# francescobrigante/Audio-Style-Transfer

Measured on AMD Instinct MI355X. Metric: audio-seconds/sec/node (train step, 4s@22.05kHz pairs), higher is better.
Workload: dtype bf16; 1 GPU; configs[1]: batch=8 4 s clips per GPU (S=2, x=(B,S,2,287,597)), full train2 step: STFT + CQT front-end from resident waveforms, encoders+decoder+discriminator, all losses, D and G phases, grad clip, Adam; global_batch=8, parallelism=dp1, hip_graph=True, dp_semantics=per-rank BN and batch-coupled losses

## Files before the change

### audio-style-transfer_amd/ast_amd/_lib.py

```python
from __future__ import annotations

import ctypes as C
import os

import torch

_HERE = os.path.dirname(os.path.abspath(__file__))
LIB_PATH = os.environ.get("AST_HIP_LIB") or os.path.join(_HERE, "libast_hip.so")

F32, BF16 = 0, 1
MAX_TAPS = 9
IGEMM_ACCUMULATE, IGEMM_RELU, IGEMM_WS_ZEROED, IGEMM_STATS, IGEMM_BN_SUMS, IGEMM_BN_NO_RELU, IGEMM_PER_IMAGE = (1 << b for b in range(7))
IGEMM_SLOTS_SHIFT, IGEMM_DET = 8, 4096

vp, i32, i64, f32 = C.c_void_p, C.c_int32, C.c_int64, C.c_float


class Gather(C.Structure):
    _fields_ = [(n, i32) for n in ("N", "Hs", "Ws", "Cs", "Hm", "Wm", "sh", "sw", "oh", "ow", "Hd", "Wd", "Cd",
                                   "dsh", "dsw", "doh", "dow", "ntaps", "wtaps")] + [("tap", i32 * MAX_TAPS)]


class WeightDesc(C.Structure):
    _fields_ = [("w", vp), ("u", vp), ("v", vp), ("sigma", vp), ("scratch", vp), ("wf", vp), ("wb", vp)] + \
# ... 10 lines not shown
    "ast_igemm": ([vp, vp, vp, vp, C.POINTER(Gather), i32, i32, vp, C.c_long, vp], i32),
    "ast_igemm_plan": ([C.POINTER(Gather), i32, C.POINTER(i32 * 5)], i32),
    "ast_pconv_variant": ([C.POINTER(Gather), i32, C.POINTER(i32 * 4)], i32),
    "ast_igemm_ws_floats": ([C.POINTER(Gather), i32], C.c_long),
    "ast_wgrad": ([vp, vp, vp, C.POINTER(Gather), i32, vp], i32),
    "ast_skinny_gemm": ([vp, vp, vp, vp, i32, i32, i32, i32, i32, i32, vp], i32),
    "ast_skinny_gemm_ex": ([vp, vp, vp, vp, i32, i32, i32, i32, i32, i32, vp, vp, f32, C.c_uint64, vp, vp], i32),
    "ast_bigk_gemm": ([vp, vp, vp, vp, i32, i32, i32, i32, vp], i32),
    "ast_bign_dgrad": ([vp, vp, vp, i32, i32, i32, i32, vp], i32),
    "ast_linear_wgrad": ([vp, vp, vp, vp, i32, i32, i32, i32, i32, vp], i32),
    "ast_linear_wgrad_batched": ([vp, i32, i32, vp], i32),
    "ast_linear_wgrad_batched_host": ([vp, i32, i32, vp], i32),
    "ast_nchw_to_nhwc": ([vp, vp, i32, i32, i32, i32, i64, i64, i64, i32, i32, vp], i32),
    "ast_nhwc_to_nchw": ([vp, vp, i32, i32, i32, i32, i32, i32, vp], i32),
    "ast_cast": ([vp, i32, vp, i32, i64, vp], i32),
    "ast_weights_prepare_t": ([vp, vp, i32, i32, i32, vp, i32, vp], i32),
    "ast_sn_scratch_floats": ([i32, i32], C.c_long),
    "ast_weight_grads_flush_t": ([vp, vp, i32, vp], i32),
    "ast_dropout_fwd": ([vp, vp, vp, i64, f32, C.c_uint64, vp, vp], i32),
    "ast_weight_grad_unpack": ([vp, i32, vp, vp, vp, vp, vp, i32, i32, i32, i32, i32, i32, i32, vp, vp], i32),
    "ast_chan_stats": ([vp, vp, i32, i32, i32, i32, i32, vp], i32),
    "ast_norm_finalize": ([vp, i32, vp, i32, i32, i32, i32, i32, vp, vp, vp, vp, i32, f32, vp, vp, vp, vp, C.c_long, vp], i32),
    "ast_affine_act": ([vp, vp, vp, vp, vp, vp, vp, i32, i32, i32, i32, i32, vp], i32),
    "ast_bn_apply_fwd": ([vp, vp, vp, vp, i32, C.c_long, vp, vp, vp, vp, vp, vp, f32, vp, vp, f32, vp, vp, i32, i32, i32, i32, i32, i32, vp], i32),
    "ast_bn_apply_bwd": ([vp, vp, vp, vp, vp, vp, i32, C.c_long, vp, vp, vp, vp, vp, vp, vp, vp, vp, vp, vp, vp, vp, vp, i32, i32, i32, i32, i32, i32, vp], i32),
    "ast_norm_bwd_sums": ([vp, vp, vp, vp, vp, i32, i32, i32, i32, i32, i32, vp], i32),
    "ast_norm_bwd_sums_pre": ([vp, vp, vp, vp, vp, i32, i32, i32, i32, i32, i32, vp, vp, vp, vp, vp], i32),
    "ast_norm_bwd_apply_pre": ([vp, vp, vp, vp, vp, vp, vp, vp, i32, i32, i32, i32, i32, vp, vp, vp, vp, vp], i32),
    "ast_norm_bwd_finalize": ([vp, i32, i32, i32, i32, i32, vp, vp, vp, vp, vp, vp, vp, vp, vp, vp, vp, vp, vp], i32),
    "ast_norm_bwd_finalize_n": ([vp, i32, i32, i32, i32, i32, vp, vp, vp, vp, vp, vp, vp, vp, vp, vp, vp, vp, C.c_long, vp], i32),
    "ast_igemm_bn": ([vp, vp, vp, vp, C.POINTER(Gather), i32, i32, vp, C.c_long, vp, vp, vp, vp], i32),
# ... 238 lines not shown
```

### audio-style-transfer_amd/ast_amd/layers.py

```python
from __future__ import annotations

import contextlib
import ctypes as C
import os

import torch
import torch.nn as nn

from . import config, ops, streams
from ._lib import LinWg, WeightDesc, check, dcode, lib, ptr, stream
from .ops import PackedWeight, pad8


class WeightBank:

    def __init__(self):
        self.specs = []
        self.entries: list[PackedWeight] = []
        self._key = None
        self._keys = {}
        self._flush_pending = False
        self._flush_stream = None
        self._lin_deferred = []
        self._pinned = []
        self._pin_pool = None
        self._pin_used = 0
        self._conv_dirty = False
        self._slab_recs = []
        self._conv_deferred = []
        self._defer_streams = []
        self._pool_flushed = False
        self._wait_lane = None
        self.d_train = self.d_eval = None
        self._dev_consts = {}
        self._packed = {}
        self.hold = False

    def add(self, weight, kind, dtype_fn, u=None, v=None, bias=None, rows=None):
        self.specs.append((weight, kind, dtype_fn, u, v, bias, rows))
        self.entries.append(PackedWeight())
        return self.entries[-1]

    def _const_dev(self, payload: bytes, dtype, dev):
        key = (payload, dtype, str(dev))
        t = self._dev_consts.get(key)
        if t is None:
            t = self._dev_consts[key] = torch.frombuffer(bytearray(payload), dtype=dtype).to(dev)
        return t
# ... 58 lines not shown
            grad_ptr = None
            if training:
                e.dwp, e.replicas, e.slab = None, rep, slab
                if sz:
                    e.dwp = self.dw_arena[off:off + sz]
                    off += sz
                    grad_ptr = ops.acc_grad(w).data_ptr() + 4 * w_off
            descs.append(WeightDesc(w=w.data_ptr() + 4 * w_off, u=ptr(u), v=ptr(v), sigma=ptr(e.sigma), scratch=ptr(e.scratch),
                                    wf=ptr(e.wf), wb=ptr(e.wb), Co=Co, Ci=Ci, KK=KK, s_co=s_co, s_ci=s_ci, Cop=e.Cop, Cip=e.Cip,
                                    power_iter=1 if training else 0, dwp=ptr(e.dwp), grad=grad_ptr, inner=ptr(e.gtmp),
                                    dwp_from_wb=1 if kind == "convT" else 0, dwp_replicas=(1 if slab else rep) if training else 1))
            dts.append(dcode(dt))
            self.max_co = max(self.max_co, Co)
            self.max_cols = max(self.max_cols, Ci * KK)
            self.max_packed = max(self.max_packed, n)
        tl = []
        for wi, e in enumerate(self.entries):
            for co0 in range(0, e.Cop, 32):
                for ci0 in range(0, e.Cip, 32):
                    tl += [wi, co0, ci0, 0]
        if self._pin_pool is None:
            self._pin_pool = torch.empty(256 * 1024, dtype=torch.uint8, pin_memory=True)
        import array
        self.ntiles = len(tl) // 4
        self.d_tiles = self._const_dev(array.array("i", tl).tobytes(), torch.int32, dev)
        arr = (WeightDesc * len(descs))(*descs)
        dev_descs = self._const_dev(bytes(arr), torch.uint8, dev)
        if training:
            self.d_train = dev_descs
        else:
            self.d_eval = dev_descs
        self.d_dtypes = self._const_dev(array.array("i", dts).tobytes(), torch.int32, dev)
        self._keys[training] = self._signature(training)

    def prepare(self, training: bool):
        if self.hold:
            return
        training = bool(training) and torch.is_grad_enabled()
        if self._keys.get(training) != self._signature(training):
            self._build(training)
        d = self.d_train if training else self.d_eval
        from . import _lib as _L
        if _L.PROFILE_CALLS is not None:
            _L.NEXT_BYTES = sum(e.Co * e.Ci * e.KK * 4 + 2 * e.wf.numel() * e.wf.element_size() for e in self.entries)
        check(lib().ast_weights_prepare_t(ptr(d), ptr(self.d_dtypes), len(self.entries), self.max_co, self.max_cols,
                                          ptr(self.d_tiles), self.ntiles, stream()), "ast_weights_prepare_t")

    def defer_linear_wgrad(self, pw, dy, x):
        self._lin_deferred.append((pw, dy, x))
        self.request_flush(conv=False)

    def defer_conv_wgrad(self, dy, src, dwp, g, replicas, pw):
        self._conv_deferred.append((dy, src, dwp, g, replicas, pw))
        if not any(b is self for b in _DeferPool.banks):
            _DeferPool.banks.append(self)

    def slab_used(self, pw):
        return next((n for p, n in self._slab_recs if p is pw), 0)

    def note_slab(self, pw, slices):
        for i, (p, n) in enumerate(self._slab_recs):
# ... 4 lines not shown

    def _sum_slabs(self):
        recs, self._slab_recs = self._slab_recs, []
        for i in range(0, len(recs), 48):
            part = recs[i:i + 48]
            n = len(part)
            bases = (C.c_void_p * n)(*[pw.dwp.data_ptr() for pw, _ in part])
            sizes = (C.c_int64 * n)(*[pw.dwp.numel() // pw.replicas for pw, _ in part])
            slabs = (C.c_int32 * n)(*[sl for _, sl in part])
            check(lib().ast_slab_sum(bases, sizes, slabs, n, stream()), "ast_slab_sum")

    def _flush_conv_kernels(self, side):
        with (torch.cuda.stream(side) if side is not None else contextlib.nullcontext()):
            if self._slab_recs:
                self._sum_slabs()
            if config.deterministic:
                ws = ops.det_ws(self.ntiles, self.d_tiles.device)
                check(lib().ast_weight_grads_flush_det(ptr(self.d_train), ptr(self.d_tiles), self.ntiles, ptr(ws), ws.numel(), stream()),
                      "ast_weight_grads_flush_det")
                return
            check(lib().ast_weight_grads_flush_t(ptr(self.d_train), ptr(self.d_tiles), self.ntiles, stream()),
                  "ast_weight_grads_flush_t")

    def _side_stream(self, origin):
        if self._flush_stream is None:
            self._flush_stream = torch.cuda.Stream(device=self.d_tiles.device)
        if not any(s is self._flush_stream for s in _ParallelFlush.pending):
            streams.fork(self._flush_stream, origin)
            _ParallelFlush.pending.append(self._flush_stream)
        return self._flush_stream

    def _launch_deferred(self, origin):
        items, self._conv_deferred = self._conv_deferred, []
        cur = torch.cuda.current_stream()
        k = max(1, min(config.wgrad_defer_streams, len(items)))
        if k > 1 and cur != origin:
# ... 20 lines not shown
    def request_flush(self, conv=True):
        self._conv_dirty = self._conv_dirty or conv
        if not self._flush_pending:
            self._flush_pending = True
            torch.autograd.Variable._execution_engine.queue_callback(self._flush)

    def _flush(self):
        self._flush_pending = False
        if ops._WgradStream.stream is not None and ops._WgradStream.dirty:
            ops._WgradStream.dirty = False
            streams.join(torch.cuda.current_stream(), ops._WgradStream.stream)
        if self._conv_dirty:
            self._conv_dirty = False
            from . import _lib as _L
            if _L.PROFILE_CALLS is not None:
                _L.NEXT_BYTES = sum((e.dwp.numel() * 4 if e.dwp is not None else 0) + 3 * e.Co * e.Ci * e.KK * 4 for e in self.entries if e.dwp is not None)
            side, origin = None, torch.cuda.current_stream()
            if _ParallelFlush.active:
                if config.wgrad_defer_pool and self._conv_deferred and len(_DeferPool.banks) > 1:
                    _DeferPool.launch_all(origin)
                side = self._side_stream(origin)
            if self._pool_flushed:
                self._pool_flushed = False
            else:
                with (torch.cuda.stream(side) if side is not None else contextlib.nullcontext()):
                    if self._conv_deferred:
                        self._launch_deferred(origin)
                    if self._wait_lane is not None:
                        torch.cuda.current_stream().wait_stream(self._wait_lane)
                        self._wait_lane = None
                self._flush_conv_kernels(side)
# ... 282 lines not shown
```

### audio-style-transfer_amd/csrc/weights.hip

```cpp
#include <type_traits>
#include "ast_common.h"
#include "../../include/ast_hip.h"

namespace {

__device__ __forceinline__ size_t woff(const ast_weight_desc_t& d, int co, int ci, int tap) {
  return (size_t)co * d.s_co + (size_t)ci * d.s_ci + tap;
}

constexpr int RZ = 32;
__global__ __launch_bounds__(256) void sn_wt_u_kernel(const ast_weight_desc_t* __restrict__ descs) {
  const ast_weight_desc_t d = descs[blockIdx.y];
  if (!d.u || !d.power_iter) return;
  const int ncols = d.Ci * d.KK;
  const int rows_per = (d.Co + RZ - 1) / RZ;
  const int c0 = blockIdx.z * rows_per, c1 = min(d.Co, c0 + rows_per);
  if (c0 >= c1) return;
  float* part = d.scratch + d.Co + (size_t)ncols * (1 + blockIdx.z);
  if (d.s_ci == d.KK && (ncols & 3) == 0 && (d.s_co & 3) == 0 && (((uintptr_t)d.w) & 15) == 0) {
    const int j4 = blockIdx.x * 256 + threadIdx.x;
    if (j4 >= (ncols >> 2)) return;
    f32x4 acc4 = {0.f, 0.f, 0.f, 0.f};
    for (int co = c0; co < c1; ++co) {
      const f32x4 w4 = *reinterpret_cast<const f32x4*>(d.w + (size_t)co * d.s_co + j4 * 4);
// ... 107 lines not shown
__device__ __forceinline__ bool tile_is_full(const ast_weight_desc_t& d, int co0, int ci0) {
  return co0 + TL <= d.Co && ci0 + TL <= d.Ci;
}
__device__ __forceinline__ bool master_vec_ok(const ast_weight_desc_t& d, const float* base) {
  const int inner = d.s_co >= d.s_ci ? d.s_ci : d.s_co, outer = d.s_co >= d.s_ci ? d.s_co : d.s_ci;
  return inner == d.KK && (outer & 3) == 0 && (((uintptr_t)base) & 15) == 0;
}

template <int KKC>
__device__ __forceinline__ void tile_load_master(const ast_weight_desc_t& d, const float* __restrict__ base, int co0, int ci0,
                                                 float* __restrict__ L, float scale) {
  const int KK = KKC > 0 ? KKC : d.KK;
  const bool co_outer = d.s_co >= d.s_ci;
  const int run = TL * KK;
  if (KKC > 0 && tile_is_full(d, co0, ci0) && master_vec_ok(d, base)) {
    const int run4 = run >> 2;
    for (int idx = threadIdx.x; idx < TL * run4; idx += 256) {
      const int o = idx / run4, r4 = idx - o * run4;
      const size_t off = co_outer ? (size_t)(co0 + o) * d.s_co + (size_t)ci0 * d.s_ci : (size_t)(ci0 + o) * d.s_ci + (size_t)co0 * d.s_co;
      const f32x4 v4 = *reinterpret_cast<const f32x4*>(base + off + r4 * 4);
#pragma unroll
      for (int e = 0; e < 4; ++e) {
        const int r = r4 * 4 + e;
        const int in = r / KK, tap = r - in * KK;
        const int co_l = co_outer ? o : in, ci_l = co_outer ? in : o;
        L[(tap * TL + co_l) * LP + ci_l] = v4[e] * scale;
      }
    }
    return;
  }
  for (int idx = threadIdx.x; idx < TL * run; idx += 256) {
    const int o = idx / run, r = idx - o * run;
    const int in = r / KK, tap = r - in * KK;
    const int co = co_outer ? co0 + o : co0 + in, ci = co_outer ? ci0 + in : ci0 + o;
    const float v = (co < d.Co && ci < d.Ci) ? base[(size_t)co * d.s_co + (size_t)ci * d.s_ci + tap] * scale : 0.f;
    L[(tap * TL + (co - co0)) * LP + (ci - ci0)] = v;
  }
}

template <typename T, int KKC>
__device__ __forceinline__ void tile_store_packed(const ast_weight_desc_t& d, int co0, int ci0, const float* __restrict__ L) {
// ... 50 lines not shown
    const float inv = 1.f / fmaxf(nrm, 1e-12f);
    sigma = nrm * nrm * inv;
    for (int i = threadIdx.x; i < d.Co; i += 256) d.u[i] = d.scratch[i] * inv;
  } else {
    float q = 0.f;
    for (int i = threadIdx.x; i < d.Co; i += 256) q += d.scratch[i] * d.u[i];
    sigma = block_sum(q, red);
  }
  if (threadIdx.x == 0) d.sigma[0] = sigma;
  __syncthreads();
}

template <int KKC>
__device__ __forceinline__ void pack_tile_body(const ast_weight_desc_t& d, const WTile& tl, int dtype, float* __restrict__ L) {
  const int KK = KKC > 0 ? KKC : d.KK;
  tile_load_master<KKC>(d, d.w, tl.co0, tl.ci0, L, 1.f / d.sigma[0]);
  __syncthreads();
  if (dtype == AST_BF16) tile_store_packed<bf16_t, KKC>(d, tl.co0, tl.ci0, L); else tile_store_packed<float, KKC>(d, tl.co0, tl.ci0, L);
  const int nrep = d.dwp_replicas > 1 ? d.dwp_replicas : 1;
  const size_t rstride = (size_t)d.Cop * KK * d.Cip;
  if (d.dwp && d.power_iter && KKC > 0 && tile_is_full(d, tl.co0, tl.ci0) && (d.Cip & 3) == 0 && (d.Cop & 3) == 0) {
    const f32x4 z = {0.f, 0.f, 0.f, 0.f};
    for (int idx = threadIdx.x; idx < TL * KK * 8; idx += 256) {
      const int q = idx & 7, row = idx >> 3;
      const int out_l = row / KK, tap = row - out_l * KK;
      float* p = d.dwp_from_wb ? d.dwp + ((size_t)(tl.ci0 + out_l) * KK + tap) * d.Cop + tl.co0 : d.dwp + ((size_t)(tl.co0 + out_l) * KK + tap) * d.Cip + tl.ci0;
      for (int r = 0; r < nrep; ++r) *reinterpret_cast<f32x4*>(p + r * rstride + q * 4) = z;
    }
  } else if (d.dwp && d.power_iter) {
    for (int idx = threadIdx.x; idx < TL * KK * TL; idx += 256) {
      const int in_l = idx & (TL - 1), row = idx >> 5;
      const int out_l = row / KK, tap = row - out_l * KK;
      for (int r = 0; r < nrep; ++r) {
        float* base = d.dwp + r * rstride;
        if (d.dwp_from_wb) { const int ci = tl.ci0 + out_l, co = tl.co0 + in_l; if (ci < d.Cip && co < d.Cop) base[((size_t)ci * KK + tap) * d.Cop + co] = 0.f; }
        else { const int co = tl.co0 + out_l, ci = tl.ci0 + in_l; if (co < d.Cop && ci < d.Cip) base[((size_t)co * KK + tap) * d.Cip + ci] = 0.f; }
      }
    }
  }
}

__global__ __launch_bounds__(256) void pack_tiles_kernel(const ast_weight_desc_t* __restrict__ descs, const int* __restrict__ dtypes,
                                                          const WTile* __restrict__ tiles) {
  __shared__ float L[9 * TL * LP];
  const WTile tl = tiles[blockIdx.x];
  const ast_weight_desc_t d = descs[tl.w];
  const int dt = dtypes[tl.w];
  if (d.KK == 9) pack_tile_body<9>(d, tl, dt, L);
  else if (d.KK == 1) pack_tile_body<1>(d, tl, dt, L);
  else pack_tile_body<0>(d, tl, dt, L);
}

template <int KKC>
__device__ __forceinline__ void tile_load_dwp(const ast_weight_desc_t& d, int co0, int ci0, float* __restrict__ G) {
  const int KK = KKC > 0 ? KKC : d.KK;
  const int nrep = d.dwp_replicas > 1 ? d.dwp_replicas : 1;
  const size_t rstride = (size_t)d.Cop * KK * d.Cip;
  if (KKC > 0 && tile_is_full(d, co0, ci0) && (d.Cip & 3) == 0 && (d.Cop & 3) == 0) {
    for (int idx = threadIdx.x; idx < TL * KK * 8; idx += 256) {
      const int q = idx & 7, row = idx >> 3;
      const int out_l = row / KK, tap = row - out_l * KK;
      const float* p = d.dwp_from_wb ? d.dwp + ((size_t)(ci0 + out_l) * KK + tap) * d.Cop + co0 : d.dwp + ((size_t)(co0 + out_l) * KK + tap) * d.Cip + ci0;
      f32x4 v4 = *reinterpret_cast<const f32x4*>(p + q * 4);
      if (nrep == 8) {
        f32x4 t[7];
#pragma unroll
        for (int r = 0; r < 7; ++r) t[r] = *reinterpret_cast<const f32x4*>(p + (r + 1) * rstride + q * 4);
        v4 = ((v4 + t[0]) + (t[1] + t[2])) + ((t[3] + t[4]) + (t[5] + t[6]));
      } else {
        for (int r = 1; r < nrep; ++r) v4 += *reinterpret_cast<const f32x4*>(p + r * rstride + q * 4);
      }
#pragma unroll
      for (int e = 0; e < 4; ++e) {
        const int in_l = q * 4 + e;
        const int co_l = d.dwp_from_wb ? in_l : out_l, ci_l = d.dwp_from_wb ? out_l : in_l;
        G[(tap * TL + co_l) * LP + ci_l] = v4[e];
      }
    }
    return;
  }
  for (int idx = threadIdx.x; idx < TL * KK * TL; idx += 256) {
    const int in_l = idx & (TL - 1), row = idx >> 5;
    const int out_l = row / KK, tap = row - out_l * KK;
    float v = 0.f;
    int co_l, ci_l;
    bool ok;
    size_t off;
    if (d.dwp_from_wb) { ci_l = out_l; co_l = in_l; const int ci = ci0 + ci_l, co = co0 + co_l; ok = ci < d.Ci && co < d.Co; off = ((size_t)ci * KK + tap) * d.Cop + co; }
    else { co_l = out_l; ci_l = in_l; const int co = co0 + co_l, ci = ci0 + ci_l; ok = co < d.Co && ci < d.Ci; off = ((size_t)co * KK + tap) * d.Cip + ci; }
    if (ok) {
      if (nrep == 8) {
        float t[8];
#pragma unroll
        for (int r = 0; r < 8; ++r) t[r] = d.dwp[r * rstride + off];
        v = ((t[0] + t[1]) + (t[2] + t[3])) + ((t[4] + t[5]) + (t[6] + t[7]));
      } else {
        for (int r = 0; r < nrep; ++r) v += d.dwp[r * rstride + off];
      }
    }
    G[(tap * TL + co_l) * LP + ci_l] = v;
  }
}

template <bool DET = false>
__global__ __launch_bounds__(256) void flush_inner_tiles_kernel(const ast_weight_desc_t* __restrict__ descs, const WTile* __restrict__ tiles,
                                                                float* __restrict__ part) {
  __shared__ float G[9 * TL * LP];
  __shared__ float red[17];
  const WTile tl = tiles[blockIdx.x];
  const ast_weight_desc_t d = descs[tl.w];
  if (!d.dwp || !d.u) {
    if constexpr (DET) { if (threadIdx.x == 0) part[blockIdx.x] = 0.f; }
    return;
  }
  float q = 0.f;
  auto body = [&](auto kkc) __attribute__((always_inline)) {
    constexpr int KKC = decltype(kkc)::value;
    const int KK = KKC > 0 ? KKC : d.KK;
    tile_load_dwp<KKC>(d, tl.co0, tl.ci0, G);
    __syncthreads();
    const bool co_outer = d.s_co >= d.s_ci;
    const int run = TL * KK;
    if (KKC > 0 && tile_is_full(d, tl.co0, tl.ci0) && master_vec_ok(d, d.w)) {
      const int run4 = run >> 2;
      for (int idx = threadIdx.x; idx < TL * run4; idx += 256) {
        const int o = idx / run4, r4 = idx - o * run4;
        const size_t off = co_outer ? (size_t)(tl.co0 + o) * d.s_co + (size_t)tl.ci0 * d.s_ci : (size_t)(tl.ci0 + o) * d.s_ci + (size_t)tl.co0 * d.s_co;
        const f32x4 w4 = *reinterpret_cast<const f32x4*>(d.w + off + r4 * 4);
#pragma unroll
        for (int e = 0; e < 4; ++e) {
          const int r = r4 * 4 + e;
          const int in = r / KK, tap = r - in * KK;
          const int co_l = co_outer ? o : in, ci_l = co_outer ? in : o;
          q += G[(tap * TL + co_l) * LP + ci_l] * w4[e];
        }
      }
      return;
    }
    for (int idx = threadIdx.x; idx < TL * run; idx += 256) {
      const int o = idx / run, r = idx - o * run;
      const int in = r / KK, tap = r - in * KK;
      const int co_l = co_outer ? o : in, ci_l = co_outer ? in : o;
      const int co = tl.co0 + co_l, ci = tl.ci0 + ci_l;
      if (co < d.Co && ci < d.Ci) q += G[(tap * TL + co_l) * LP + ci_l] * d.w[(size_t)co * d.s_co + (size_t)ci * d.s_ci + tap];
    }
  };
  if (d.KK == 9) body(std::integral_constant<int, 9>{});
  else if (d.KK == 1) body(std::integral_constant<int, 1>{});
  else body(std::integral_constant<int, 0>{});
  q = block_sum(q, red);
  if constexpr (DET) {
    if (threadIdx.x == 0) part[blockIdx.x] = q / d.sigma[0];
  } else {
    if (threadIdx.x == 0 && q != 0.f) unsafeAtomicAdd(d.inner, q / d.sigma[0]);
  }
}

__global__ __launch_bounds__(256) void inner_sum_det_kernel(const ast_weight_desc_t* __restrict__ descs, const WTile* __restrict__ tiles,
                                                            const float* __restrict__ part, int ntiles) {
  const int t = blockIdx.x * 256 + threadIdx.x;
  if (t >= ntiles) return;
  const int w = tiles[t].w;
  if (t > 0 && tiles[t - 1].w == w) return;
  const ast_weight_desc_t d = descs[w];
  if (!d.dwp || !d.u) return;
  float v = 0.f;
  for (int i = t; i < ntiles && tiles[i].w == w; ++i) v += part[i];
  d.inner[0] = v;
}

__global__ __launch_bounds__(256) void flush_unpack_tiles_kernel(const ast_weight_desc_t* __restrict__ descs, const WTile* __restrict__ tiles) {
  __shared__ float G[9 * TL * LP];
  const WTile tl = tiles[blockIdx.x];
  const ast_weight_desc_t d = descs[tl.w];
  if (!d.dwp || !d.grad) return;
  const float inner = d.u ? d.inner[0] : 0.f;
  const float inv_sigma = d.u ? 1.f / d.sigma[0] : 1.f;
  auto body = [&](auto kkc) __attribute__((always_inline)) {
    constexpr int KKC = decltype(kkc)::value;
    const int KK = KKC > 0 ? KKC : d.KK;
    tile_load_dwp<KKC>(d, tl.co0, tl.ci0, G);
    __syncthreads();
    const bool co_outer = d.s_co >= d.s_ci;
    const int run = TL * KK;
    if (KKC > 0 && tile_is_full(d, tl.co0, tl.ci0) && master_vec_ok(d, d.grad)) {
      const int run4 = run >> 2;
      for (int idx = threadIdx.x; idx < TL * run4; idx += 256) {
        const int o = idx / run4, r4 = idx - o * run4;
        const size_t off = co_outer ? (size_t)(tl.co0 + o) * d.s_co + (size_t)tl.ci0 * d.s_ci : (size_t)(tl.ci0 + o) * d.s_ci + (size_t)tl.co0 * d.s_co;
        f32x4* gp = reinterpret_cast<f32x4*>(d.grad + off + r4 * 4);
        f32x4 g4 = *gp;
#pragma unroll
        for (int e = 0; e < 4; ++e) {
          const int r = r4 * 4 + e;
          const int in = r / KK, tap = r - in * KK;
          const int co_l = co_outer ? o : in, ci_l = co_outer ? in : o;
          float gv = G[(tap * TL + co_l) * LP + ci_l];
          if (d.u) gv = (gv - inner * d.u[tl.co0 + co_l] * d.v[(tl.ci0 + ci_l) * KK + tap]) * inv_sigma;
          g4[e] += gv;
        }
        *gp = g4;
      }
      return;
    }
    for (int idx = threadIdx.x; idx < TL * run; idx += 256) {
      const int o = idx / run, r = idx - o * run;
      const int in = r / KK, tap = r - in * KK;
      const int co_l = co_outer ? o : in, ci_l = co_outer ? in : o;
      const int co = tl.co0 + co_l, ci = tl.ci0 + ci_l;
      if (co < d.Co && ci < d.Ci) {
        float gv = G[(tap * TL + co_l) * LP + ci_l];
        if (d.u) gv = (gv - inner * d.u[co] * d.v[ci * KK + tap]) * inv_sigma;
        d.grad[(size_t)co * d.s_co + (size_t)ci * d.s_ci + tap] += gv;
      }
    }
  };
  if (d.KK == 9) body(std::integral_constant<int, 9>{});
  else if (d.KK == 1) body(std::integral_constant<int, 1>{});
  else body(std::integral_constant<int, 0>{});
}
}

extern "C" int ast_weights_prepare_t(const ast_weight_desc_t* descs, const int* dtypes, int n, int max_co, int max_cols,
                                     const void* tiles, int ntiles, void* stream) {
  if (!descs || !dtypes || !tiles || n <= 0 || ntiles <= 0 || max_co <= 0 || max_cols <= 0) AST_FAIL("ast_weights_prepare_t: bad args");
  hipStream_t s = (hipStream_t)stream;
  hipLaunchKernelGGL(sn_wt_u_kernel, dim3((max_cols + 255) / 256, n, RZ), dim3(256), 0, s, descs);
  hipLaunchKernelGGL(sn_t_sum_kernel, dim3((max_cols + 255) / 256, n), dim3(256), 0, s, descs);
  hipLaunchKernelGGL(sn_w_v_kernel, dim3((max_co + 3) / 4, n), dim3(256), 0, s, descs);
  hipLaunchKernelGGL(sn_sigma_kernel, dim3(n), dim3(256), 0, s, descs);
  hipLaunchKernelGGL(pack_tiles_kernel, dim3(ntiles), dim3(256), 0, s, descs, dtypes, (const WTile*)tiles);
  AST_CHECK_LAUNCH();
  return 0;
}

extern "C" int ast_weight_grads_flush_t(const ast_weight_desc_t* descs, const void* tiles, int ntiles, void* stream) {
  if (!descs || !tiles || ntiles <= 0) AST_FAIL("ast_weight_grads_flush_t: bad args");
  hipStream_t s = (hipStream_t)stream;
  hipLaunchKernelGGL(flush_inner_tiles_kernel<false>, dim3(ntiles), dim3(256), 0, s, descs, (const WTile*)tiles, (float*)nullptr);
  hipLaunchKernelGGL(flush_unpack_tiles_kernel, dim3(ntiles), dim3(256), 0, s, descs, (const WTile*)tiles);
  AST_CHECK_LAUNCH();
  return 0;
}

extern "C" int ast_weight_grads_flush_det(const ast_weight_desc_t* descs, const void* tiles, int ntiles, float* ws, long ws_floats, void* stream) {
  if (!descs || !tiles || !ws || ntiles <= 0 || ws_floats < ntiles) AST_FAIL("ast_weight_grads_flush_det: bad args (ws >= ntiles floats)");
  hipStream_t s = (hipStream_t)stream;
  hipLaunchKernelGGL(flush_inner_tiles_kernel<true>, dim3(ntiles), dim3(256), 0, s, descs, (const WTile*)tiles, ws);
  hipLaunchKernelGGL(inner_sum_det_kernel, dim3((ntiles + 255) / 256), dim3(256), 0, s, descs, (const WTile*)tiles, (const float*)ws, ntiles);
  hipLaunchKernelGGL(flush_unpack_tiles_kernel, dim3(ntiles), dim3(256), 0, s, descs, (const WTile*)tiles);
  AST_CHECK_LAUNCH();
  return 0;
}

extern "C" int ast_weight_grad_unpack(const float* dwp, int from_wb, const float* w, const float* u, const float* v,
                                      const float* sigma, float* g_orig, int Co, int Ci, int KK, int s_co, int s_ci, int Cop,
                                      int Cip, float* scratch, void* stream) {
  if (!dwp || !w || !g_orig || (u && (!v || !sigma || !scratch))) AST_FAIL("ast_weight_grad_unpack: bad args");
  hipStream_t s = (hipStream_t)stream;
  const size_t n = (size_t)Co * Ci * KK;
  const int nb = (int)std::max<size_t>(1, std::min<size_t>(512, (n + 1023) / 1024));
  if (u) {
    AST_HIP(hipMemsetAsync(scratch, 0, sizeof(float), s));
    hipLaunchKernelGGL(wgrad_inner_kernel, dim3(nb), dim3(256), 0, s, dwp, from_wb, w, sigma, scratch, Co, Ci, KK, s_co, s_ci, Cop, Cip);
  }
// ... 11 lines not shown
```

### include/ast_hip.h

```cpp
#ifndef AST_HIP_H
#define AST_HIP_H
#include <stddef.h>
#include <stdint.h>
#ifdef __cplusplus
extern "C" {
#endif

#define AST_DTYPE_F32 0
#define AST_DTYPE_BF16 1
#define AST_MAX_TAPS 9

int ast_version(void);
const char* ast_last_error(void);

typedef struct ast_gather_t {
  int32_t N, Hs, Ws, Cs;
  int32_t Hm, Wm;
  int32_t sh, sw, oh, ow;
  int32_t Hd, Wd, Cd;
  int32_t dsh, dsw, doh, dow;
  int32_t ntaps, wtaps;
  int32_t tap[AST_MAX_TAPS];
} ast_gather_t;

// ... 47 lines not shown
  float* v;
  float* sigma;
  float* scratch;
  void* wf;
  void* wb;
  int32_t Co, Ci, KK, s_co, s_ci, Cop, Cip;
  int32_t power_iter;
  float* dwp;
  float* grad;
  float* inner;
  int32_t dwp_from_wb;
  int32_t dwp_replicas;
} ast_weight_desc_t;
long ast_sn_scratch_floats(int Co, int ncols);
int ast_weights_prepare_t(const ast_weight_desc_t* descs, const int* dtypes, int n, int max_co, int max_cols,
                          const void* tiles, int ntiles, void* stream);
int ast_weight_grads_flush_t(const ast_weight_desc_t* descs, const void* tiles, int ntiles, void* stream);
int ast_weight_grad_unpack(const float* dwp, int from_wb, const float* w, const float* u, const float* v,
                           const float* sigma, float* g_orig, int Co, int Ci, int KK, int s_co, int s_ci,
                           int Cop, int Cip, float* scratch, void* stream);

int ast_chan_stats(const void* x, float* sums, int N, int HW, int C, int dtype, int assume_zeroed, void* stream);
int ast_norm_finalize(float* sums, int zero_sums, int64_t* num_batches_tracked ,
                      int N, int HW, int C, int Creal, int instance,
                      const float* gamma, const float* beta, float* running_mean, float* running_var,
                      int eval_mode, float eps, float* mean, float* rstd, float* scale, float* shift,
                      long count, void* stream);
int ast_affine_act(const void* x, const float* scale, const float* shift, const void* r,
                   const float* scale2, const float* shift2, void* y, int N, int HW, int C,
                   int flags, int dtype, void* stream);
int ast_bn_apply_fwd(const void* x, const void* r, void* y, const float* tab1, int rows1, long count1, const float* tab2,
// ... 274 lines not shown
```

Measured before the change: 5373 audio-seconds/sec.

## Specialize weight pack/flush kernels by tap count and fuse replica reduction into flush

Sorts the weight tiles by kernel size (3x3, 1x1, other) and launches a separate templated pack kernel per class, so LDS size and loops are fixed at compile time. Weights without gradients are dropped from the flush tile list. The flush's first pass now sums the replica gradients and writes the sum back, so the second (unpack) pass reads a single replica and skips non-spectral-norm weights. Loads are batched into registers before the LDS writes, and the dwp zeroing moves ahead of the pack. This adds code complexity and more kernel launches in exchange for less redundant memory traffic in the weight prepare and flush stages.

```diff
diff --git a/audio-style-transfer_amd/ast_amd/_lib.py b/audio-style-transfer_amd/ast_amd/_lib.py
--- a/audio-style-transfer_amd/ast_amd/_lib.py
+++ b/audio-style-transfer_amd/ast_amd/_lib.py
@@ -48,7 +48,7 @@
     "ast_nchw_to_nhwc": ([vp, vp, i32, i32, i32, i32, i64, i64, i64, i32, i32, vp], i32),
     "ast_nhwc_to_nchw": ([vp, vp, i32, i32, i32, i32, i32, i32, vp], i32),
     "ast_cast": ([vp, i32, vp, i32, i64, vp], i32),
-    "ast_weights_prepare_t": ([vp, vp, i32, i32, i32, vp, i32, vp], i32),
+    "ast_weights_prepare_t": ([vp, vp, i32, i32, i32, vp, i32, i32, i32, vp], i32),
     "ast_sn_scratch_floats": ([i32, i32], C.c_long),
     "ast_weight_grads_flush_t": ([vp, vp, i32, vp], i32),
     "ast_dropout_fwd": ([vp, vp, vp, i64, f32, C.c_uint64, vp, vp], i32),
diff --git a/audio-style-transfer_amd/ast_amd/layers.py b/audio-style-transfer_amd/ast_amd/layers.py
--- a/audio-style-transfer_amd/ast_amd/layers.py
+++ b/audio-style-transfer_amd/ast_amd/layers.py
@@ -32,6 +32,7 @@
         self._pool_flushed = False
         self._wait_lane = None
         self.d_train = self.d_eval = None
+        self.d_flush_tiles, self.n_flush_tiles = None, 0
         self._dev_consts = {}
         self._packed = {}
         self.hold = False
@@ -120,16 +121,12 @@
             self.max_co = max(self.max_co, Co)
             self.max_cols = max(self.max_cols, Ci * KK)
             self.max_packed = max(self.max_packed, n)
-        tl = []
-        for wi, e in enumerate(self.entries):
-            for co0 in range(0, e.Cop, 32):
-                for ci0 in range(0, e.Cip, 32):
-                    tl += [wi, co0, ci0, 0]
+        self.d_tiles, self.ntiles, self.n9, self.n1 = self._tile_list(self.entries, lambda e: True, dev)
+        if training:
+            self.d_flush_tiles, self.n_flush_tiles, _, _ = self._tile_list(self.entries, lambda e: e.dwp is not None, dev)
         if self._pin_pool is None:
             self._pin_pool = torch.empty(256 * 1024, dtype=torch.uint8, pin_memory=True)
         import array
-        self.ntiles = len(tl) // 4
-        self.d_tiles = self._const_dev(array.array("i", tl).tobytes(), torch.int32, dev)
         arr = (WeightDesc * len(descs))(*descs)
         dev_descs = self._const_dev(bytes(arr), torch.uint8, dev)
         if training:
@@ -138,6 +135,45 @@
             self.d_eval = dev_descs
         self.d_dtypes = self._const_dev(array.array("i", dts).tobytes(), torch.int32, dev)
         self._keys[training] = self._signature(training)
+
+    @staticmethod
+    def tile_order(kks):
+        cls = lambda kk: 0 if kk == 9 else 1 if kk == 1 else 2
+        return sorted(range(len(kks)), key=lambda i: (cls(kks[i]), i))
+
+    def _tile_list(self, entries, keep, dev):
+        import array
+        tl, counts = [], [0, 0, 0]
+        for wi in self.tile_order([e.KK for e in entries]):
+            e = entries[wi]
+            if e.KK > 9:
+                raise ValueError(f"WeightBank: {e.KK} taps; the tiled pack / flush kernels hold at most 9 (3x3)")
+            if not keep(e):
+                continue
+            for co0 in range(0, e.Cop, 32):
+                for ci0 in range(0, e.Cip, 32):
+                    tl += [wi, co0, ci0, 0]
+                    counts[0 if e.KK == 9 else 1 if e.KK == 1 else 2] += 1
+        n = len(tl) // 4
+        return (self._const_dev(array.array("i", tl).tobytes(), torch.int32, dev) if n else None), n, counts[0], counts[1]
+
+    def pack_bytes(self, training):
+        return sum(e.Co * e.Ci * e.KK * 4 + 2 * e.wf.numel() * e.wf.element_size()
+                   + (e.Cop * e.KK * e.Cip * 4 * (1 if e.slab else e.replicas) if training and e.dwp is not None else 0)
+                   for e in self.entries)
+
+    def flush_bytes(self):
+        tot = 0
+        for e in self.entries:
+            if e.dwp is None:
+                continue
+            one, n = e.Cop * e.KK * e.Cip * 4, e.Co * e.Ci * e.KK * 4
+            rep = 1 if e.slab else e.replicas
+            if e.u is None:
+                tot += one * rep + 2 * n
+            else:
+                tot += one * rep + n + (one if rep > 1 else 0) + one + 2 * n
+        return tot
 
     def prepare(self, training: bool):
         if self.hold:
@@ -148,9 +184,9 @@
         d = self.d_train if training else self.d_eval
         from . import _lib as _L
         if _L.PROFILE_CALLS is not None:
-            _L.NEXT_BYTES = sum(e.Co * e.Ci * e.KK * 4 + 2 * e.wf.numel() * e.wf.element_size() for e in self.entries)
+            _L.NEXT_BYTES = self.pack_bytes(training)
         check(lib().ast_weights_prepare_t(ptr(d), ptr(self.d_dtypes), len(self.entries), self.max_co, self.max_cols,
-                                          ptr(self.d_tiles), self.ntiles, stream()), "ast_weights_prepare_t")
+                                          ptr(self.d_tiles), self.ntiles, self.n9, self.n1, stream()), "ast_weights_prepare_t")
 
     def defer_linear_wgrad(self, pw, dy, x):
         self._lin_deferred.append((pw, dy, x))
@@ -185,12 +221,14 @@
         with (torch.cuda.stream(side) if side is not None else contextlib.nullcontext()):
             if self._slab_recs:
                 self._sum_slabs()
+            if not self.n_flush_tiles:
+                return
             if config.deterministic:
-                ws = ops.det_ws(self.ntiles, self.d_tiles.device)
-                check(lib().ast_weight_grads_flush_det(ptr(self.d_train), ptr(self.d_tiles), self.ntiles, ptr(ws), ws.numel(), stream()),
-                      "ast_weight_grads_flush_det")
+                ws = ops.det_ws(self.n_flush_tiles, self.d_tiles.device)
+                check(lib().ast_weight_grads_flush_det(ptr(self.d_train), ptr(self.d_flush_tiles), self.n_flush_tiles, ptr(ws), ws.numel(),
+                                                       stream()), "ast_weight_grads_flush_det")
                 return
-            check(lib().ast_weight_grads_flush_t(ptr(self.d_train), ptr(self.d_tiles), self.ntiles, stream()),
+            check(lib().ast_weight_grads_flush_t(ptr(self.d_train), ptr(self.d_flush_tiles), self.n_flush_tiles, stream()),
                   "ast_weight_grads_flush_t")
 
     def _side_stream(self, origin):
@@ -241,7 +279,7 @@
             self._conv_dirty = False
             from . import _lib as _L
             if _L.PROFILE_CALLS is not None:
-                _L.NEXT_BYTES = sum((e.dwp.numel() * 4 if e.dwp is not None else 0) + 3 * e.Co * e.Ci * e.KK * 4 for e in self.entries if e.dwp is not None)
+                _L.NEXT_BYTES = self.flush_bytes()
             side, origin = None, torch.cuda.current_stream()
             if _ParallelFlush.active:
                 if config.wgrad_defer_pool and self._conv_deferred and len(_DeferPool.banks) > 1:
diff --git a/audio-style-transfer_amd/csrc/weights.hip b/audio-style-transfer_amd/csrc/weights.hip
--- a/audio-style-transfer_amd/csrc/weights.hip
+++ b/audio-style-transfer_amd/csrc/weights.hip
@@ -145,17 +145,30 @@
   const bool co_outer = d.s_co >= d.s_ci;
   const int run = TL * KK;
   if (KKC > 0 && tile_is_full(d, co0, ci0) && master_vec_ok(d, base)) {
-    const int run4 = run >> 2;
-    for (int idx = threadIdx.x; idx < TL * run4; idx += 256) {
-      const int o = idx / run4, r4 = idx - o * run4;
-      const size_t off = co_outer ? (size_t)(co0 + o) * d.s_co + (size_t)ci0 * d.s_ci : (size_t)(ci0 + o) * d.s_ci + (size_t)co0 * d.s_co;
-      const f32x4 v4 = *reinterpret_cast<const f32x4*>(base + off + r4 * 4);
-#pragma unroll
-      for (int e = 0; e < 4; ++e) {
-        const int r = r4 * 4 + e;
-        const int in = r / KK, tap = r - in * KK;
-        const int co_l = co_outer ? o : in, ci_l = co_outer ? in : o;
-        L[(tap * TL + co_l) * LP + ci_l] = v4[e] * scale;
+    constexpr int run4 = (TL * (KKC > 0 ? KKC : 1)) >> 2;
+    constexpr int NIT = (TL * run4 + 255) / 256;
+    f32x4 v4[NIT];
+#pragma unroll
+    for (int it = 0; it < NIT; ++it) {
+      const int idx = threadIdx.x + it * 256;
+      if (idx < TL * run4) {
+        const int o = idx / run4, r4 = idx - o * run4;
+        const size_t off = co_outer ? (size_t)(co0 + o) * d.s_co + (size_t)ci0 * d.s_ci : (size_t)(ci0 + o) * d.s_ci + (size_t)co0 * d.s_co;
+        v4[it] = *reinterpret_cast<const f32x4*>(base + off + r4 * 4);
+      }
+    }
+#pragma unroll
+    for (int it = 0; it < NIT; ++it) {
+      const int idx = threadIdx.x + it * 256;
+      if (idx < TL * run4) {
+        const int o = idx / run4, r4 = idx - o * run4;
+#pragma unroll
+        for (int e = 0; e < 4; ++e) {
+          const int r = r4 * 4 + e;
+          const int in = r / KK, tap = r - in * KK;
+          const int co_l = co_outer ? o : in, ci_l = co_outer ? in : o;
+          L[(tap * TL + co_l) * LP + ci_l] = v4[it][e] * scale;
+        }
       }
     }
     return;
@@ -236,19 +249,15 @@
 template <int KKC>
 __device__ __forceinline__ void pack_tile_body(const ast_weight_desc_t& d, const WTile& tl, int dtype, float* __restrict__ L) {
   const int KK = KKC > 0 ? KKC : d.KK;
-  tile_load_master<KKC>(d, d.w, tl.co0, tl.ci0, L, 1.f / d.sigma[0]);
-  __syncthreads();
-  if (dtype == AST_BF16) tile_store_packed<bf16_t, KKC>(d, tl.co0, tl.ci0, L); else tile_store_packed<float, KKC>(d, tl.co0, tl.ci0, L);
   const int nrep = d.dwp_replicas > 1 ? d.dwp_replicas : 1;
   const size_t rstride = (size_t)d.Cop * KK * d.Cip;
   if (d.dwp && d.power_iter && KKC > 0 && tile_is_full(d, tl.co0, tl.ci0) && (d.Cip & 3) == 0 && (d.Cop & 3) == 0) {
     const f32x4 z = {0.f, 0.f, 0.f, 0.f};
-    for (int idx = threadIdx.x; idx < TL * KK * 8; idx += 256) {
-      const int q = idx & 7, row = idx >> 3;
-      const int out_l = row / KK, tap = row - out_l * KK;
-      float* p = d.dwp_from_wb ? d.dwp + ((size_t)(tl.ci0 + out_l) * KK + tap) * d.Cop + tl.co0 : d.dwp + ((size_t)(tl.co0 + out_l) * KK + tap) * d.Cip + tl.ci0;
-      for (int r = 0; r < nrep; ++r) *reinterpret_cast<f32x4*>(p + r * rstride + q * 4) = z;
-    }
+    const int ld = d.dwp_from_wb ? d.Cop : d.Cip;
+    float* p0 = d.dwp_from_wb ? d.dwp + (size_t)tl.ci0 * KK * ld + tl.co0 : d.dwp + (size_t)tl.co0 * KK * ld + tl.ci0;
+    for (int r = 0; r < nrep; ++r)
+      for (int idx = threadIdx.x; idx < TL * KK * 8; idx += 256)
+        *reinterpret_cast<f32x4*>(p0 + r * rstride + (size_t)(idx >> 3) * ld + (idx & 7) * 4) = z;
   } else if (d.dwp && d.power_iter) {
     for (int idx = threadIdx.x; idx < TL * KK * TL; idx += 256) {
       const int in_l = idx & (TL - 1), row = idx >> 5;
@@ -260,44 +269,67 @@
       }
     }
   }
-}
-
+  tile_load_master<KKC>(d, d.w, tl.co0, tl.ci0, L, 1.f / d.sigma[0]);
+  __syncthreads();
+  if (dtype == AST_BF16) tile_store_packed<bf16_t, KKC>(d, tl.co0, tl.ci0, L); else tile_store_packed<float, KKC>(d, tl.co0, tl.ci0, L);
+}
+
+template <int KKC>
 __global__ __launch_bounds__(256) void pack_tiles_kernel(const ast_weight_desc_t* __restrict__ descs, const int* __restrict__ dtypes,
                                                           const WTile* __restrict__ tiles) {
-  __shared__ float L[9 * TL * LP];
+  __shared__ float L[(KKC > 0 ? KKC : 9) * TL * LP];
   const WTile tl = tiles[blockIdx.x];
   const ast_weight_desc_t d = descs[tl.w];
-  const int dt = dtypes[tl.w];
-  if (d.KK == 9) pack_tile_body<9>(d, tl, dt, L);
-  else if (d.KK == 1) pack_tile_body<1>(d, tl, dt, L);
-  else pack_tile_body<0>(d, tl, dt, L);
-}
-
-template <int KKC>
-__device__ __forceinline__ void tile_load_dwp(const ast_weight_desc_t& d, int co0, int ci0, float* __restrict__ G) {
+  if (KKC > 0 ? d.KK != KKC : d.KK > 9) return;
+  pack_tile_body<KKC>(d, tl, dtypes[tl.w], L);
+}
+
+template <int KKC, bool WRITE_SUM>
+__device__ __forceinline__ void tile_load_dwp(const ast_weight_desc_t& d, int co0, int ci0, float* __restrict__ G, int nrep_in) {
   const int KK = KKC > 0 ? KKC : d.KK;
-  const int nrep = d.dwp_replicas > 1 ? d.dwp_replicas : 1;
+  const int nrep = nrep_in > 0 ? nrep_in : (d.dwp_replicas > 1 ? d.dwp_replicas : 1);
   const size_t rstride = (size_t)d.Cop * KK * d.Cip;
   if (KKC > 0 && tile_is_full(d, co0, ci0) && (d.Cip & 3) == 0 && (d.Cop & 3) == 0) {
-    for (int idx = threadIdx.x; idx < TL * KK * 8; idx += 256) {
+    const int ld = d.dwp_from_wb ? d.Cop : d.Cip;
+    float* p0 = d.dwp_from_wb ? d.dwp + (size_t)ci0 * KK * ld + co0 : d.dwp + (size_t)co0 * KK * ld + ci0;
+    auto to_lds = [&](int idx, const f32x4& v4) __attribute__((always_inline)) {
       const int q = idx & 7, row = idx >> 3;
       const int out_l = row / KK, tap = row - out_l * KK;
-      const float* p = d.dwp_from_wb ? d.dwp + ((size_t)(ci0 + out_l) * KK + tap) * d.Cop + co0 : d.dwp + ((size_t)(co0 + out_l) * KK + tap) * d.Cip + ci0;
-      f32x4 v4 = *reinterpret_cast<const f32x4*>(p + q * 4);
-      if (nrep == 8) {
-        f32x4 t[7];
-#pragma unroll
-        for (int r = 0; r < 7; ++r) t[r] = *reinterpret_cast<const f32x4*>(p + (r + 1) * rstride + q * 4);
-        v4 = ((v4 + t[0]) + (t[1] + t[2])) + ((t[3] + t[4]) + (t[5] + t[6]));
-      } else {
-        for (int r = 1; r < nrep; ++r) v4 += *reinterpret_cast<const f32x4*>(p + r * rstride + q * 4);
-      }
 #pragma unroll
       for (int e = 0; e < 4; ++e) {
         const int in_l = q * 4 + e;
         const int co_l = d.dwp_from_wb ? in_l : out_l, ci_l = d.dwp_from_wb ? out_l : in_l;
         G[(tap * TL + co_l) * LP + ci_l] = v4[e];
       }
+    };
+    if (nrep == 1) {
+      constexpr int NIT = (TL * (KKC > 0 ? KKC : 1) * 8 + 255) / 256;
+      f32x4 v[NIT];
+#pragma unroll
+      for (int it = 0; it < NIT; ++it) {
+        const int idx = threadIdx.x + it * 256;
+        if (idx < TL * KK * 8) v[it] = *reinterpret_cast<const f32x4*>(p0 + (size_t)(idx >> 3) * ld + (idx & 7) * 4);
+      }
+#pragma unroll
+      for (int it = 0; it < NIT; ++it) {
+        const int idx = threadIdx.x + it * 256;
+        if (idx < TL * KK * 8) to_lds(idx, v[it]);
+      }
+      return;
+    }
+    for (int idx = threadIdx.x; idx < TL * KK * 8; idx += 256) {
+      float* p = p0 + (size_t)(idx >> 3) * ld + (idx & 7) * 4;
+      f32x4 v4 = *reinterpret_cast<const f32x4*>(p);
+      if (nrep == 8) {
+        f32x4 t[7];
+#pragma unroll
+        for (int r = 0; r < 7; ++r) t[r] = *reinterpret_cast<const f32x4*>(p + (r + 1) * rstride);
+        v4 = ((v4 + t[0]) + (t[1] + t[2])) + ((t[3] + t[4]) + (t[5] + t[6]));
+      } else {
+        for (int r = 1; r < nrep; ++r) v4 += *reinterpret_cast<const f32x4*>(p + r * rstride);
+      }
+      if (WRITE_SUM) *reinterpret_cast<f32x4*>(p) = v4;
+      to_lds(idx, v4);
     }
     return;
   }
@@ -319,57 +351,136 @@
       } else {
         for (int r = 0; r < nrep; ++r) v += d.dwp[r * rstride + off];
       }
+      if (WRITE_SUM && nrep > 1) d.dwp[off] = v;
     }
     G[(tap * TL + co_l) * LP + ci_l] = v;
   }
 }
 
+__device__ __forceinline__ size_t master_run_off(const ast_weight_desc_t& d, int co0, int ci0, int o) {
+  return d.s_co >= d.s_ci ? (size_t)(co0 + o) * d.s_co + (size_t)ci0 * d.s_ci : (size_t)(ci0 + o) * d.s_ci + (size_t)co0 * d.s_co;
+}
+
+template <int KKC>
+__device__ __forceinline__ float tile_inner(const ast_weight_desc_t& d, int co0, int ci0, const float* __restrict__ G) {
+  const int KK = KKC > 0 ? KKC : d.KK;
+  const bool co_outer = d.s_co >= d.s_ci;
+  const int run = TL * KK;
+  float q = 0.f;
+  if (KKC > 0 && tile_is_full(d, co0, ci0) && master_vec_ok(d, d.w)) {
+    constexpr int run4 = (TL * (KKC > 0 ? KKC : 1)) >> 2;
+    constexpr int NIT = (TL * run4 + 255) / 256;
+    f32x4 w4[NIT];
+#pragma unroll
+    for (int it = 0; it < NIT; ++it) {
+      const int idx = threadIdx.x + it * 256;
+      if (idx < TL * run4) { const int o = idx / run4; w4[it] = *reinterpret_cast<const f32x4*>(d.w + master_run_off(d, co0, ci0, o) + (idx - o * run4) * 4); }
+    }
+#pragma unroll
+    for (int it = 0; it < NIT; ++it) {
+      const int idx = threadIdx.x + it * 256;
+      if (idx < TL * run4) {
+        const int o = idx / run4, r4 = idx - o * run4;
+#pragma unroll
+        for (int e = 0; e < 4; ++e) {
+          const int r = r4 * 4 + e;
+          const int in = r / KK, tap = r - in * KK;
+          const int co_l = co_outer ? o : in, ci_l = co_outer ? in : o;
+          q += G[(tap * TL + co_l) * LP + ci_l] * w4[it][e];
+        }
+      }
+    }
+    return q;
+  }
+  for (int idx = threadIdx.x; idx < TL * run; idx += 256) {
+    const int o = idx / run, r = idx - o * run;
+    const int in = r / KK, tap = r - in * KK;
+    const int co_l = co_outer ? o : in, ci_l = co_outer ? in : o;
+    const int co = co0 + co_l, ci = ci0 + ci_l;
+    if (co < d.Co && ci < d.Ci) q += G[(tap * TL + co_l) * LP + ci_l] * d.w[(size_t)co * d.s_co + (size_t)ci * d.s_ci + tap];
+  }
+  return q;
+}
+
+template <int KKC>
+__device__ __forceinline__ void tile_unpack(const ast_weight_desc_t& d, int co0, int ci0, const float* __restrict__ G, float inner,
+                                            float inv_sigma) {
+  const int KK = KKC > 0 ? KKC : d.KK;
+  const bool co_outer = d.s_co >= d.s_ci;
+  const int run = TL * KK;
+  if (KKC > 0 && tile_is_full(d, co0, ci0) && master_vec_ok(d, d.grad)) {
+    constexpr int run4 = (TL * (KKC > 0 ? KKC : 1)) >> 2;
+    constexpr int NIT = (TL * run4 + 255) / 256;
+    f32x4 g4[NIT];
+#pragma unroll
+    for (int it = 0; it < NIT; ++it) {
+      const int idx = threadIdx.x + it * 256;
+      if (idx < TL * run4) { const int o = idx / run4; g4[it] = *reinterpret_cast<const f32x4*>(d.grad + master_run_off(d, co0, ci0, o) + (idx - o * run4) * 4); }
+    }
+#pragma unroll
+    for (int it = 0; it < NIT; ++it) {
+      const int idx = threadIdx.x + it * 256;
+      if (idx < TL * run4) {
+        const int o = idx / run4, r4 = idx - o * run4;
+        f32x4 g = g4[it];
+#pragma unroll
+        for (int e = 0; e < 4; ++e) {
+          const int r = r4 * 4 + e;
+          const int in = r / KK, tap = r - in * KK;
+          const int co_l = co_outer ? o : in, ci_l = co_outer ? in : o;
+          float gv = G[(tap * TL + co_l) * LP + ci_l];
+          if (d.u) gv = (gv - inner * d.u[co0 + co_l] * d.v[(ci0 + ci_l) * KK + tap]) * inv_sigma;
+          g[e] += gv;
+        }
+        *reinterpret_cast<f32x4*>(d.grad + master_run_off(d, co0, ci0, o) + r4 * 4) = g;
+      }
+    }
+    return;
+  }
+  for (int idx = threadIdx.x; idx < TL * run; idx += 256) {
+    const int o = idx / run, r = idx - o * run;
+    const int in = r / KK, tap = r - in * KK;
+    const int co_l = co_outer ? o : in, ci_l = co_outer ? in : o;
+    const int co = co0 + co_l, ci = ci0 + ci_l;
+    if (co < d.Co && ci < d.Ci) {
+      float gv = G[(tap * TL + co_l) * LP + ci_l];
+      if (d.u) gv = (gv - inner * d.u[co] * d.v[ci * KK + tap]) * inv_sigma;
+      d.grad[(size_t)co * d.s_co + (size_t)ci * d.s_ci + tap] += gv;
+    }
+  }
+}
+
 template <bool DET = false>
-__global__ __launch_bounds__(256) void flush_inner_tiles_kernel(const ast_weight_desc_t* __restrict__ descs, const WTile* __restrict__ tiles,
-                                                                float* __restrict__ part) {
+__global__ __launch_bounds__(256) void flush_first_kernel(const ast_weight_desc_t* __restrict__ descs, const WTile* __restrict__ tiles,
+                                                          float* __restrict__ part) {
   __shared__ float G[9 * TL * LP];
   __shared__ float red[17];
   const WTile tl = tiles[blockIdx.x];
   const ast_weight_desc_t d = descs[tl.w];
-  if (!d.dwp || !d.u) {
+  if (!d.dwp || d.KK > 9 || (!d.u && !d.grad)) {
     if constexpr (DET) { if (threadIdx.x == 0) part[blockIdx.x] = 0.f; }
     return;
   }
   float q = 0.f;
   auto body = [&](auto kkc) __attribute__((always_inline)) {
     constexpr int KKC = decltype(kkc)::value;
-    const int KK = KKC > 0 ? KKC : d.KK;
-    tile_load_dwp<KKC>(d, tl.co0, tl.ci0, G);
+    if (!d.u) {
+      tile_load_dwp<KKC, false>(d, tl.co0, tl.ci0, G, 0);
+      __syncthreads();
+      tile_unpack<KKC>(d, tl.co0, tl.ci0, G, 0.f, 1.f);
+      return;
+    }
+    tile_load_dwp<KKC, true>(d, tl.co0, tl.ci0, G, 0);
     __syncthreads();
-    const bool co_outer = d.s_co >= d.s_ci;
-    const int run = TL * KK;
-    if (KKC > 0 && tile_is_full(d, tl.co0, tl.ci0) && master_vec_ok(d, d.w)) {
-      const int run4 = run >> 2;
-      for (int idx = threadIdx.x; idx < TL * run4; idx += 256) {
-        const int o = idx / run4, r4 = idx - o * run4;
-        const size_t off = co_outer ? (size_t)(tl.co0 + o) * d.s_co + (size_t)tl.ci0 * d.s_ci : (size_t)(tl.ci0 + o) * d.s_ci + (size_t)tl.co0 * d.s_co;
-        const f32x4 w4 = *reinterpret_cast<const f32x4*>(d.w + off + r4 * 4);
-#pragma unroll
-        for (int e = 0; e < 4; ++e) {
-          const int r = r4 * 4 + e;
-          const int in = r / KK, tap = r - in * KK;
-          const int co_l = co_outer ? o : in, ci_l = co_outer ? in : o;
-          q += G[(tap * TL + co_l) * LP + ci_l] * w4[e];
-        }
-      }
-      return;
-    }
-    for (int idx = threadIdx.x; idx < TL * run; idx += 256) {
-      const int o = idx / run, r = idx - o * run;
-      const int in = r / KK, tap = r - in * KK;
-      const int co_l = co_outer ? o : in, ci_l = co_outer ? in : o;
-      const int co = tl.co0 + co_l, ci = tl.ci0 + ci_l;
-      if (co < d.Co && ci < d.Ci) q += G[(tap * TL + co_l) * LP + ci_l] * d.w[(size_t)co * d.s_co + (size_t)ci * d.s_ci + tap];
-    }
+    q = tile_inner<KKC>(d, tl.co0, tl.ci0, G);
   };
   if (d.KK == 9) body(std::integral_constant<int, 9>{});
   else if (d.KK == 1) body(std::integral_constant<int, 1>{});
   else body(std::integral_constant<int, 0>{});
+  if (!d.u) {
+    if constexpr (DET) { if (threadIdx.x == 0) part[blockIdx.x] = 0.f; }
+    return;
+  }
   q = block_sum(q, red);
   if constexpr (DET) {
     if (threadIdx.x == 0) part[blockIdx.x] = q / d.sigma[0];
@@ -391,51 +502,18 @@
   d.inner[0] = v;
 }
 
-__global__ __launch_bounds__(256) void flush_unpack_tiles_kernel(const ast_weight_desc_t* __restrict__ descs, const WTile* __restrict__ tiles) {
+__global__ __launch_bounds__(256) void flush_unpack_sn_kernel(const ast_weight_desc_t* __restrict__ descs, const WTile* __restrict__ tiles) {
   __shared__ float G[9 * TL * LP];
   const WTile tl = tiles[blockIdx.x];
   const ast_weight_desc_t d = descs[tl.w];
-  if (!d.dwp || !d.grad) return;
-  const float inner = d.u ? d.inner[0] : 0.f;
-  const float inv_sigma = d.u ? 1.f / d.sigma[0] : 1.f;
+  if (!d.dwp || !d.grad || !d.u || d.KK > 9) return;
+  const float inner = d.inner[0];
+  const float inv_sigma = 1.f / d.sigma[0];
   auto body = [&](auto kkc) __attribute__((always_inline)) {
     constexpr int KKC = decltype(kkc)::value;
-    const int KK = KKC > 0 ? KKC : d.KK;
-    tile_load_dwp<KKC>(d, tl.co0, tl.ci0, G);
+    tile_load_dwp<KKC, false>(d, tl.co0, tl.ci0, G, 1);
     __syncthreads();
-    const bool co_outer = d.s_co >= d.s_ci;
-    const int run = TL * KK;
-    if (KKC > 0 && tile_is_full(d, tl.co0, tl.ci0) && master_vec_ok(d, d.grad)) {
-      const int run4 = run >> 2;
-      for (int idx = threadIdx.x; idx < TL * run4; idx += 256) {
-        const int o = idx / run4, r4 = idx - o * run4;
-        const size_t off = co_outer ? (size_t)(tl.co0 + o) * d.s_co + (size_t)tl.ci0 * d.s_ci : (size_t)(tl.ci0 + o) * d.s_ci + (size_t)tl.co0 * d.s_co;
-        f32x4* gp = reinterpret_cast<f32x4*>(d.grad + off + r4 * 4);
-        f32x4 g4 = *gp;
-#pragma unroll
-        for (int e = 0; e < 4; ++e) {
-          const int r = r4 * 4 + e;
-          const int in = r / KK, tap = r - in * KK;
-          const int co_l = co_outer ? o : in, ci_l = co_outer ? in : o;
-          float gv = G[(tap * TL + co_l) * LP + ci_l];
-          if (d.u) gv = (gv - inner * d.u[tl.co0 + co_l] * d.v[(tl.ci0 + ci_l) * KK + tap]) * inv_sigma;
-          g4[e] += gv;
-        }
-        *gp = g4;
-      }
-      return;
-    }
-    for (int idx = threadIdx.x; idx < TL * run; idx += 256) {
-      const int o = idx / run, r = idx - o * run;
-      const int in = r / KK, tap = r - in * KK;
-      const int co_l = co_outer ? o : in, ci_l = co_outer ? in : o;
-      const int co = tl.co0 + co_l, ci = tl.ci0 + ci_l;
-      if (co < d.Co && ci < d.Ci) {
-        float gv = G[(tap * TL + co_l) * LP + ci_l];
-        if (d.u) gv = (gv - inner * d.u[co] * d.v[ci * KK + tap]) * inv_sigma;
-        d.grad[(size_t)co * d.s_co + (size_t)ci * d.s_ci + tap] += gv;
-      }
-    }
+    tile_unpack<KKC>(d, tl.co0, tl.ci0, G, inner, inv_sigma);
   };
   if (d.KK == 9) body(std::integral_constant<int, 9>{});
   else if (d.KK == 1) body(std::integral_constant<int, 1>{});
@@ -444,14 +522,18 @@
 }
 
 extern "C" int ast_weights_prepare_t(const ast_weight_desc_t* descs, const int* dtypes, int n, int max_co, int max_cols,
-                                     const void* tiles, int ntiles, void* stream) {
-  if (!descs || !dtypes || !tiles || n <= 0 || ntiles <= 0 || max_co <= 0 || max_cols <= 0) AST_FAIL("ast_weights_prepare_t: bad args");
+                                     const void* tiles, int ntiles, int n9, int n1, void* stream) {
+  if (!descs || !dtypes || !tiles || n <= 0 || ntiles <= 0 || max_co <= 0 || max_cols <= 0 || n9 < 0 || n1 < 0 || n9 + n1 > ntiles)
+    AST_FAIL("ast_weights_prepare_t: bad args");
   hipStream_t s = (hipStream_t)stream;
+  const WTile* tl = (const WTile*)tiles;
   hipLaunchKernelGGL(sn_wt_u_kernel, dim3((max_cols + 255) / 256, n, RZ), dim3(256), 0, s, descs);
   hipLaunchKernelGGL(sn_t_sum_kernel, dim3((max_cols + 255) / 256, n), dim3(256), 0, s, descs);
   hipLaunchKernelGGL(sn_w_v_kernel, dim3((max_co + 3) / 4, n), dim3(256), 0, s, descs);
   hipLaunchKernelGGL(sn_sigma_kernel, dim3(n), dim3(256), 0, s, descs);
-  hipLaunchKernelGGL(pack_tiles_kernel, dim3(ntiles), dim3(256), 0, s, descs, dtypes, (const WTile*)tiles);
+  if (n9) hipLaunchKernelGGL(pack_tiles_kernel<9>, dim3(n9), dim3(256), 0, s, descs, dtypes, tl);
+  if (n1) hipLaunchKernelGGL(pack_tiles_kernel<1>, dim3(n1), dim3(256), 0, s, descs, dtypes, tl + n9);
+  if (ntiles - n9 - n1) hipLaunchKernelGGL(pack_tiles_kernel<0>, dim3(ntiles - n9 - n1), dim3(256), 0, s, descs, dtypes, tl + n9 + n1);
   AST_CHECK_LAUNCH();
   return 0;
 }
@@ -459,8 +541,8 @@
 extern "C" int ast_weight_grads_flush_t(const ast_weight_desc_t* descs, const void* tiles, int ntiles, void* stream) {
   if (!descs || !tiles || ntiles <= 0) AST_FAIL("ast_weight_grads_flush_t: bad args");
   hipStream_t s = (hipStream_t)stream;
-  hipLaunchKernelGGL(flush_inner_tiles_kernel<false>, dim3(ntiles), dim3(256), 0, s, descs, (const WTile*)tiles, (float*)nullptr);
-  hipLaunchKernelGGL(flush_unpack_tiles_kernel, dim3(ntiles), dim3(256), 0, s, descs, (const WTile*)tiles);
+  hipLaunchKernelGGL(flush_first_kernel<false>, dim3(ntiles), dim3(256), 0, s, descs, (const WTile*)tiles, (float*)nullptr);
+  hipLaunchKernelGGL(flush_unpack_sn_kernel, dim3(ntiles), dim3(256), 0, s, descs, (const WTile*)tiles);
   AST_CHECK_LAUNCH();
   return 0;
 }
@@ -468,9 +550,9 @@
 extern "C" int ast_weight_grads_flush_det(const ast_weight_desc_t* descs, const void* tiles, int ntiles, float* ws, long ws_floats, void* stream) {
   if (!descs || !tiles || !ws || ntiles <= 0 || ws_floats < ntiles) AST_FAIL("ast_weight_grads_flush_det: bad args (ws >= ntiles floats)");
   hipStream_t s = (hipStream_t)stream;
-  hipLaunchKernelGGL(flush_inner_tiles_kernel<true>, dim3(ntiles), dim3(256), 0, s, descs, (const WTile*)tiles, ws);
+  hipLaunchKernelGGL(flush_first_kernel<true>, dim3(ntiles), dim3(256), 0, s, descs, (const WTile*)tiles, ws);
   hipLaunchKernelGGL(inner_sum_det_kernel, dim3((ntiles + 255) / 256), dim3(256), 0, s, descs, (const WTile*)tiles, (const float*)ws, ntiles);
-  hipLaunchKernelGGL(flush_unpack_tiles_kernel, dim3(ntiles), dim3(256), 0, s, descs, (const WTile*)tiles);
+  hipLaunchKernelGGL(flush_unpack_sn_kernel, dim3(ntiles), dim3(256), 0, s, descs, (const WTile*)tiles);
   AST_CHECK_LAUNCH();
   return 0;
 }
diff --git a/include/ast_hip.h b/include/ast_hip.h
--- a/include/ast_hip.h
+++ b/include/ast_hip.h
@@ -85,7 +85,7 @@
 } ast_weight_desc_t;
 long ast_sn_scratch_floats(int Co, int ncols);
 int ast_weights_prepare_t(const ast_weight_desc_t* descs, const int* dtypes, int n, int max_co, int max_cols,
-                          const void* tiles, int ntiles, void* stream);
+                          const void* tiles, int ntiles, int n9, int n1, void* stream);
 int ast_weight_grads_flush_t(const ast_weight_desc_t* descs, const void* tiles, int ntiles, void* stream);
 int ast_weight_grad_unpack(const float* dwp, int from_wb, const float* w, const float* u, const float* v,
                            const float* sigma, float* g_orig, int Co, int Ci, int KK, int s_co, int s_ci,
```

After: 5300 audio-seconds/sec. 0.986x the previous value.
